# qq456cvb/VoteNet

Measured on AMD Instinct MI355X. Metric: SUN RGB-D 20k-pt scenes/sec (fwd+bwd), higher is better.
Workload: dtype f32

## Files before the change

### __graft_entry__.py

```python
import os
import sys

ROOT = os.path.dirname(os.path.abspath(__file__))
if ROOT not in sys.path:
    sys.path.insert(0, ROOT)


def build():
    import votenet_amd
    path = votenet_amd.build()
    from votenet_amd import _lib
    _lib.lib()
    _lib.monitors_lib()
    _lib.guard_lib()
    _lib.features_lib()
    _lib.detect_lib()
    _lib.boxpts_lib()
    _lib.aabb_lib()
    from oracle import oracle as O
    O.build()
    O.lib()
    print("built", path)


def smoke():
    import numpy as np
    import torch
    from oracle import oracle as O
    from votenet_amd import tf_grouping, tf_interpolate, tf_sampling
    assert torch.cuda.is_available(), "smoke() needs a GPU"
    dev = torch.device("cuda:0")
    xyz = np.random.default_rng(0).random((2, 2048, 3), dtype=np.float32)
    x = torch.from_numpy(xyz).to(dev)
    fidx = tf_sampling.farthest_point_sample(512, x)
    assert (fidx.cpu().numpy() == O.farthest_point_sample(512, xyz)).all(), "FPS indices differ from the oracle"
    new_xyz = tf_sampling.gather_point(x, fidx)
    idx, cnt = tf_grouping.query_ball_point(0.2, 32, x, new_xyz)
    oi, oc = O.query_ball_point(0.2, 32, xyz, new_xyz.cpu().numpy())
    assert (idx.cpu().numpy() == oi).all() and (cnt.cpu().numpy() == oc).all(), "ball query differs from the oracle"
    g = tf_grouping.group_point(x, idx)
    assert (g.cpu().numpy() == O.group_point(xyz, oi)).all(), "group_point differs from the oracle"
    dist, nn = tf_interpolate.three_nn(x, new_xyz)
    od, on = O.three_nn(xyz, new_xyz.cpu().numpy())
    assert (nn.cpu().numpy() == on).all() and (dist.cpu().numpy() == od).all(), "three_nn differs from the oracle"
    from votenet_amd import mlp
    rng = np.random.default_rng(1)
    w0 = (rng.normal(size=(6, 64)) * 0.5).astype(np.float32)
    w1 = (rng.normal(size=(64, 64)) * 0.2).astype(np.float32)
    ones, zeros = np.ones(64, np.float32), np.zeros(64, np.float32)
    a = O.group_concat(xyz, new_xyz.cpu().numpy(), xyz, oi).reshape(-1, 6)
    for w in (w0, w1):
        zz = O.linear(a, w, zeros)
        mean, var = O.bn_stats(zz)
        a = O.bn_relu(zz, mean, var, ones, zeros)
    exp = O.max_over_k(a, 32)
    T = lambda v: torch.from_numpy(v).to(dev)
    rows = 2 * 512 * 32
    z, st = mlp.linear_gather(x, new_xyz, x, idx, T(w0), T(zeros))
    sc, sh, _, _ = mlp.bn_finalize(rows, st, T(ones), T(zeros))
    z, st = mlp.linear_dense(z, T(w1), T(zeros), sc, sh, True)
    sc, sh, _, _ = mlp.bn_finalize(rows, st, T(ones), T(zeros))
    got, _ = mlp.bn_relu_max(z, 32, sc, sh, True)
    err = float(np.abs(got.cpu().numpy() - exp).max() / max(1.0, np.abs(exp).max()))
    assert err < 1e-5, "grouped MLP differs from the oracle: %g" % err
    z0, st0 = mlp.linear_gather(x, new_xyz, x, idx, T(w0), T(zeros))
    sc0, sh0, _, _ = mlp.bn_finalize(rows, st0, T(ones), T(zeros))
    w1d = T(w1)
    img = mlp.SplitImages([w1d])
    img.refresh()
    z3, st3 = mlp.linear_dense(z0, w1d, T(zeros), sc0, sh0, True)
    img.close()
# ... 37 lines not shown
```

### votenet_amd/_lib.py

```python
import ctypes
import os
import re
import subprocess

import torch

_HERE = os.path.dirname(os.path.abspath(__file__))
_LIB_PATH = os.path.join(_HERE, "lib", "libvotenet_hip.so")
_MON_PATH = os.path.join(_HERE, "lib", "libvotenet_monitors.so")
_GUARD_PATH = os.path.join(_HERE, "lib", "libvotenet_guard.so")
_FEAT_PATH = os.path.join(_HERE, "lib", "libvotenet_features.so")
_lib = None
_mon = None
_guard = None
_feat = None
_DETECT_PATH = os.path.join(_HERE, "lib", "libvotenet_detect.so")
_detect = None
_BOXPTS_PATH = os.path.join(_HERE, "lib", "libvotenet_boxpts.so")
_boxpts = None
_AABB_PATH = os.path.join(_HERE, "lib", "libvotenet_aabb.so")
_aabb = None


class VotenetError(RuntimeError):
    """A HIP runtime / launch / workspace error reported by libvotenet_hip.so."""


class InvalidArgumentError(ValueError):
    """Mirror of tf.errors.InvalidArgumentError raised by the reference's OP_REQUIRES checks."""


def lib_path():
    return _LIB_PATH


def build(force=False):
    if force:
        import glob
        mon = os.path.join(os.path.dirname(_LIB_PATH), os.path.basename(_MON_PATH))
        guard = os.path.join(os.path.dirname(_LIB_PATH), os.path.basename(_GUARD_PATH))
        feat = os.path.join(os.path.dirname(_LIB_PATH), os.path.basename(_FEAT_PATH))
        detect = os.path.join(os.path.dirname(_LIB_PATH), os.path.basename(_DETECT_PATH))
        boxpts = os.path.join(os.path.dirname(_LIB_PATH), os.path.basename(_BOXPTS_PATH))
        aabb = os.path.join(os.path.dirname(_LIB_PATH), os.path.basename(_AABB_PATH))
        for f in [_LIB_PATH, mon, guard, feat, detect, boxpts, aabb] + [o for d in ("obj", os.path.join("monitors", "obj"), os.path.join("guard", "obj"), os.path.join("features", "obj"),
                                                                               os.path.join("detect", "obj"), os.path.join("boxpts", "obj"), os.path.join("aabb", "obj"))
                                            for o in glob.glob(os.path.join(_HERE, "csrc", d, "*.o"))]:
            if os.path.exists(f):
                os.remove(f)
    out = subprocess.run(["bash", os.path.join(_HERE, "csrc", "build.sh")], capture_output=True, text=True)
    if out.returncode != 0:
        raise VotenetError("libvotenet_hip.so build failed:\n" + out.stdout + out.stderr)
    return _LIB_PATH


_SCALARS = {"int": ctypes.c_int, "long": ctypes.c_long, "float": ctypes.c_float, "double": ctypes.c_double, "unsigned": ctypes.c_uint,
            "unsigned long long": ctypes.c_ulonglong, "size_t": ctypes.c_size_t}
_POINTEES = set(_SCALARS) | {"void", "char", "unsigned char", "unsigned short", "long long"}


def _declarator(text, where):
    words = text.replace("*", " * ").split()
    if not words or not words[-1].isidentifier():
        raise ValueError("%s: cannot read the declaration '%s'" % (where, " ".join(text.split())))
    return " ".join(w for w in words[:-1] if w != "const" and w != "*"), words.count("*"), words[-1]


def _ctype(base, stars, structs, where, ret=False):
    if stars == 0 and base in _SCALARS:
        return _SCALARS[base]
    if stars == 0 and ret and base == "void":
        return None
    if stars == 1 and base in structs:
        return ctypes.POINTER(structs[base])
    if stars == 1 and ret and base == "char":
        return ctypes.c_char_p
    if stars == 1 and base in _POINTEES:
        return ctypes.c_void_p
    raise ValueError("%s: no ctypes type for the C type '%s'" % (where, base + " *" * stars))


def parse_header(text, structs):
    text = re.sub(r"/\*.*?\*/|//[^\n]*", " ", text, flags=re.S)
    text = re.sub(r"#ifdef __cplusplus.*?#endif", "", text, flags=re.S)
    text = re.sub(r"^[ \t]*#.*$", "", text, flags=re.M)

    def struct(m):
        name, fields = m.group(2), []
        for line in filter(str.strip, m.group(1).split(";")):
            decls = [_declarator(d, name) for d in line.split(",")]
            fields += [(n, _ctype(decls[0][0], stars, structs, name + "." + n)) for _, stars, n in decls]
        structs[name] = type("".join(w.capitalize() for w in name.split("_")[1:]), (ctypes.Structure,),
                             {"_fields_": fields, "__doc__": "struct %s of the C ABI." % name})
        return ""
    text = re.sub(r"typedef\s+struct\s+\w+\s*\{(.*?)\}\s*(\w+)\s*;", struct, text, flags=re.S)
    funcs = {}
    for stmt in text.split(";"):
        if not stmt.strip():
            continue
# ... 102 lines not shown
            fn.restype, fn.argtypes = restype, argtypes
        _feat = F
    return _feat


def detect_lib():
    global _detect
    if _detect is None:
        if not os.path.exists(_DETECT_PATH):
            raise VotenetError("libvotenet_detect.so not found at %s -- run `python -c 'import __graft_entry__ as g; g.build()'` "
                               "(there is no CPU fallback)" % _DETECT_PATH)
        with open(os.path.join(_HERE, os.pardir, "include", "votenet_detections.h")) as f:
            protos = parse_header(f.read(), {})
        D = ctypes.CDLL(_DETECT_PATH)
        for name, (restype, argtypes) in protos.items():
            fn = getattr(D, name)
            fn.restype, fn.argtypes = restype, argtypes
        _detect = D
    return _detect


def boxpts_lib():
    global _boxpts
    if _boxpts is None:
        if not os.path.exists(_BOXPTS_PATH):
            raise VotenetError("libvotenet_boxpts.so not found at %s -- run `python -c 'import __graft_entry__ as g; g.build()'` "
                               "(there is no CPU fallback)" % _BOXPTS_PATH)
        with open(os.path.join(_HERE, os.pardir, "include", "votenet_box_points.h")) as f:
            protos = parse_header(f.read(), {})
        B = ctypes.CDLL(_BOXPTS_PATH)
        for name, (restype, argtypes) in protos.items():
            fn = getattr(B, name)
            fn.restype, fn.argtypes = restype, argtypes
        _boxpts = B
    return _boxpts


def aabb_lib():
    global _aabb
    if _aabb is None:
        if not os.path.exists(_AABB_PATH):
            raise VotenetError("libvotenet_aabb.so not found at %s -- run `python -c 'import __graft_entry__ as g; g.build()'` "
                               "(there is no CPU fallback)" % _AABB_PATH)
        with open(os.path.join(_HERE, os.pardir, "include", "votenet_aabb_nms.h")) as f:
            protos = parse_header(f.read(), {})
        A = ctypes.CDLL(_AABB_PATH)
        for name, (restype, argtypes) in protos.items():
            fn = getattr(A, name)
            fn.restype, fn.argtypes = restype, argtypes
        _aabb = A
    return _aabb


def check_aabb(rc):
    if rc == 0:
        return
    msg = aabb_lib().votenet_aabb_last_error().decode()
    if rc == 1:
        raise InvalidArgumentError(msg)
    raise VotenetError("libvotenet_aabb error %d: %s" % (rc, msg))


def check_boxpts(rc):
    if rc == 0:
        return
    msg = boxpts_lib().votenet_box_points_last_error().decode()
    if rc == 1:
        raise InvalidArgumentError(msg)
    raise VotenetError("libvotenet_boxpts error %d: %s" % (rc, msg))


def check_detect(rc):
    if rc == 0:
        return
    msg = detect_lib().votenet_detections_last_error().decode()
    if rc == 1:
        raise InvalidArgumentError(msg)
    raise VotenetError("libvotenet_detect error %d: %s" % (rc, msg))


def check_features(rc):
    if rc == 0:
        return
    msg = features_lib().votenet_point_features_last_error().decode()
    if rc == 1:
        raise InvalidArgumentError(msg)
    raise VotenetError("libvotenet_features error %d: %s" % (rc, msg))


def check_guard(rc):
    if rc == 0:
        return
    msg = guard_lib().votenet_step_guard_last_error().decode()
    if rc == 1:
        raise InvalidArgumentError(msg)
    raise VotenetError("libvotenet_guard error %d: %s" % (rc, msg))


def check_monitors(rc):
    if rc == 0:
        return
    msg = monitors_lib().votenet_monitors_last_error().decode()
    if rc == 1:
        raise InvalidArgumentError(msg)
    raise VotenetError("libvotenet_monitors error %d: %s" % (rc, msg))

# ... 67 lines not shown
```

### votenet_amd/csrc/grouping.hip

```cpp
#include "common.h"
#include <cmath>

namespace votenet {


template <int NW, int G = 8>
__global__ __launch_bounds__(NW * 64) void ball_query_kernel(int n, int m, float thr, int nsample,
                                                              const float *__restrict__ xyz1,
                                                              const float *__restrict__ xyz2, int *__restrict__ idx,
                                                              int *__restrict__ pts_cnt)
{
    constexpr int WPQ = NW * G;
    constexpr int CHUNK = WPQ * 32;
    constexpr int QPW = 64 / NW;
    constexpr int LPQ = WPQ / 64 > 0 ? WPQ / 64 : 1;
    __shared__ unsigned masks[64][WPQ + 1];

    const int scene = blockIdx.y;
    const float *__restrict__ cand = xyz1 + (size_t)scene * n * 3;
    const float *__restrict__ qry = xyz2 + (size_t)scene * m * 3;
    int *__restrict__ oidx = idx + (size_t)scene * m * nsample;
    int *__restrict__ ocnt = pts_cnt + (size_t)scene * m;

    const int lane = lane_id();
    const int w = wave_id_uniform();
    const int q0 = blockIdx.x * 64;
    const int q = q0 + lane;
    const bool qvalid = q < m;
    const int qq = qvalid ? q : (m - 1);
    const float qx = qry[(size_t)qq * 3 + 0], qy = qry[(size_t)qq * 3 + 1], qz = qry[(size_t)qq * 3 + 2];

    int cnt[QPW];
    int first[QPW];
#pragma unroll
    for (int i = 0; i < QPW; i++) {
        cnt[i] = 0;
        first[i] = 0;
    }

    for (int base = 0; base < n; base += CHUNK) {
#pragma unroll 1
        for (int g = 0; g < G; g++) {
            const int wbase = __builtin_amdgcn_readfirstlane(base + (w * G + g) * 32);
            unsigned mask = 0;
            if (wbase < n) {
                const int valid = (n - wbase) < 32 ? (n - wbase) : 32;
                if (valid == 32) {
#pragma unroll
                    for (int t = 0; t < 32; t++) {
                        const float cx = cand[(size_t)(wbase + t) * 3 + 0];
                        const float cy = cand[(size_t)(wbase + t) * 3 + 1];
                        const float cz = cand[(size_t)(wbase + t) * 3 + 2];
                        const float dx = qx - cx, dy = qy - cy, dz = qz - cz;
// ... 59 lines not shown
            if (cnt[i] < nsample && q0 + ql < m) wave_full = false;
        }
        if (__syncthreads_and(wave_full ? 1 : 0)) break;
    }
#pragma unroll
    for (int i = 0; i < QPW; i++) {
        const int ql = w * QPW + i;
        if (q0 + ql < m) {
            const int c = cnt[i] < nsample ? cnt[i] : nsample;
            int *__restrict__ row = oidx + (size_t)(q0 + ql) * nsample;
            for (int l = c + lane; l < nsample; l += 64) row[l] = first[i];
            if (lane == 0) ocnt[q0 + ql] = c;
        }
    }
}

__global__ void group_point_vec4_kernel(long rows, int n, int c4, long rows_per_scene, const float4 *__restrict__ points,
                                        const int *__restrict__ idx, float4 *__restrict__ out)
{
    const long total = rows * c4;
    for (long e = (long)blockIdx.x * blockDim.x + threadIdx.x; e < total; e += (long)gridDim.x * blockDim.x) {
        const long row = e / c4;
        const int v = (int)(e - row * c4);
        const long s = row / rows_per_scene;
        const int ii = idx[row];
        out[e] = points[((size_t)s * n + ii) * c4 + v];
    }
}

__global__ void group_point_kernel(long rows, int n, int c, long rows_per_scene, const float *__restrict__ points,
                                   const int *__restrict__ idx, float *__restrict__ out)
{
    const long total = rows * c;
    for (long e = (long)blockIdx.x * blockDim.x + threadIdx.x; e < total; e += (long)gridDim.x * blockDim.x) {
        const long row = e / c;
        const int l = (int)(e - row * c);
        const long s = row / rows_per_scene;
        const int ii = idx[row];
        out[e] = points[((size_t)s * n + ii) * c + l];
    }
}

__global__ void group_point_grad_kernel(long rows, int n, int c, long rows_per_scene, const float *__restrict__ grad_out,
                                        const int *__restrict__ idx, float *__restrict__ grad_points)
{
    const long total = rows * c;
    for (long e = (long)blockIdx.x * blockDim.x + threadIdx.x; e < total; e += (long)gridDim.x * blockDim.x) {
        const long row = e / c;
        const int l = (int)(e - row * c);
        const long s = row / rows_per_scene;
        const int ii = idx[row];
        unsafeAtomicAdd(&grad_points[((size_t)s * n + ii) * c + l], grad_out[e]);
    }
}

float ball_threshold(float r)
{
    float t = r * r;
    while (t > 0.0f && sqrtf(t) >= r) t = nextafterf(t, 0.0f);
    while (sqrtf(t) < r) t = nextafterf(t, INFINITY);
    return t;
}

static inline int grid_for(long total, int block)
{
    long g = (total + block - 1) / block;
    if (g > 256 * 16) g = 256 * 16;
    if (g < 1) g = 1;
    return (int)g;
}

}

using namespace votenet;

extern "C" float votenet_ball_threshold(float radius) { return ball_threshold(radius); }

static int g_bq_small = 0;
extern "C" void votenet_debug_ball_query_small(int form) { VN_DEBUG_GATE(); g_bq_small = form; }

extern "C" int votenet_query_ball_point(int b, int n, int m, float radius, int nsample, const float *xyz1,
                                        const float *xyz2, int *idx, int *pts_cnt, void *stream)
{
    VN_REQUIRE(radius > 0, "QueryBallPoint expects positive radius");
    VN_REQUIRE(nsample > 0, "QueryBallPoint expects positive nsample");
    VN_REQUIRE(b >= 0 && n > 0, "QueryBallPoint expects (batch_size, ndataset, 3) xyz1 shape.");
    VN_REQUIRE(m >= 0, "QueryBallPoint expects (batch_size, npoint, 3) xyz2 shape.");
    if (b == 0 || m == 0) return VOTENET_OK;
    VN_REQUIRE(xyz1 && xyz2 && idx && pts_cnt, "QueryBallPoint: null buffer");
    const float thr = (radius <= 1e-20f) ? -1.0f : ball_threshold(radius);
    hipStream_t st = as_stream(stream);
    dim3 grid((m + 63) / 64, b);
    if (n > 2048 || g_bq_small == 16)
        hipLaunchKernelGGL((ball_query_kernel<16>), grid, dim3(1024), 0, st, n, m, thr, nsample, xyz1, xyz2, idx, pts_cnt);
    else if (g_bq_small == 4)
        hipLaunchKernelGGL((ball_query_kernel<4>), grid, dim3(256), 0, st, n, m, thr, nsample, xyz1, xyz2, idx, pts_cnt);
    else if (n > 1024)
        hipLaunchKernelGGL((ball_query_kernel<16, 4>), grid, dim3(1024), 0, st, n, m, thr, nsample, xyz1, xyz2, idx, pts_cnt);
    else if (n > 512)
        hipLaunchKernelGGL((ball_query_kernel<16, 2>), grid, dim3(1024), 0, st, n, m, thr, nsample, xyz1, xyz2, idx, pts_cnt);
    else
        hipLaunchKernelGGL((ball_query_kernel<16, 1>), grid, dim3(1024), 0, st, n, m, thr, nsample, xyz1, xyz2, idx, pts_cnt);
    return check_launch("query_ball_point");
}

namespace votenet {
constexpr int BQI_CH = 6;
constexpr int BQI_U = 6;
template <int WAVES>
__global__ __launch_bounds__(WAVES * 64) void ball_query_indexed_kernel(int n, int m, float thr, int nsample,
                                                                        const float *__restrict__ xyz2, const int *__restrict__ perm,
                                                                        const float *__restrict__ bbox,
                                                                        const float4 *__restrict__ sorted, int *__restrict__ idx,
                                                                        int *__restrict__ pts_cnt)
// ... 173 lines not shown
```

### votenet_amd/mlp.py

```python
import ctypes

import torch

from . import _lib as L

PROFILE_EVENTS = None
PROFILE_SHAPES = None


class _Timed:
    def __init__(self, kind, flops, shape=None, limit=None):
        self.kind, self.flops, self.shape = kind, flops, shape
        if limit is not None and getattr(limit, "nh_limit", None) is not None:
            self.flops = (flops, limit.nh_dev, BALL_PIECES * limit.G)

    def __enter__(self):
        if PROFILE_EVENTS is not None:
            self.e0, self.e1 = torch.cuda.Event(enable_timing=True), torch.cuda.Event(enable_timing=True)
            self.e0.record()

    def __exit__(self, *a):
        if PROFILE_EVENTS is not None:
            self.e1.record()
            PROFILE_EVENTS.append((self.e0, self.e1, self.kind, self.flops) if PROFILE_SHAPES is None else (self.e0, self.e1, self.kind, self.flops, self.shape))
# ... 520 lines not shown


def assemble_rows_half(xyz, new_xyz, idx, pts_cnt, half):
    b, m, k = idx.shape
    n = xyz.shape[1]
    if k != 64:
        raise L.InvalidArgumentError("assemble_rows_half expects nsample == 64")
    geo = torch.empty((b * m * 64, 4), dtype=torch.float32, device=xyz.device)
    npts = b * n
    nz = npts * 4 + 16 + (npts + 1) // 2
    if half.nh_limit is not None and _StatsArena.active and _StatsArena.whole_step:
        zero = _zeros_i64((nz,), xyz.device)
    else:
        zero = torch.zeros(nz, dtype=torch.int64, device=xyz.device)
    cntv = zero[:npts * 4].view(npts, 4)
    mom = zero[npts * 4:npts * 4 + 9].view(torch.float64)
    work = zero[npts * 4 + 16:].view(torch.int32)[:npts]
    with L.device_guard(xyz.device):
        L.check(L.lib().votenet_assemble_rows_half(b, n, m, L.ptr(half.nh_dev), L.ptr(xyz), L.ptr(new_xyz), L.ptr(idx), L.ptr(pts_cnt),
                                                   L.ptr(half._hc), L.ptr(geo), L.ptr(cntv), L.ptr(mom), L.ptr(work), L.stream_ptr()))
    half._geo, half._work = geo, work
    return geo, cntv, mom


def narrow_rows_half(xyz, new_xyz, feat, idx, pts_cnt, half):
    b, m, k = idx.shape
    n = xyz.shape[1]
    c = feat.shape[2] if feat is not None else 0
    if k != 64:
        raise L.InvalidArgumentError("narrow_rows_half expects nsample == 64")
    u8 = torch.empty((b * m * 64, 8), dtype=torch.float32, device=xyz.device)
    mom = torch.zeros(72, dtype=torch.float64, device=xyz.device)
    with L.device_guard(xyz.device):
        L.check(L.lib().votenet_narrow_rows_half(b, n, m, c, L.ptr(half.nh_dev), L.ptr(xyz), L.ptr(new_xyz), L.ptr(feat), L.ptr(idx),
                                                 L.ptr(pts_cnt), L.ptr(half._hc), L.ptr(u8), L.ptr(mom), L.stream_ptr()))
    half._u8 = u8
    return u8, mom


def half_sort_rows(half, npts):
    dev = half._geo.device
    work, half._work = getattr(half, "_work", None), None
    counted = work is not None
    if not counted:
        work = torch.empty(npts, dtype=torch.int32, device=dev)
    order = torch.empty(half.G * 64, dtype=torch.int32, device=dev)
    with L.device_guard(dev):
        L.check(L.lib().votenet_half_sort_rows(npts, half.G, L.ptr(half.nh_dev), L.ptr(half._geo), L.ptr(work), 1 if counted else 0, L.ptr(order),
                                               L.stream_ptr()))
    half._order = order
    if half.nh is not None:
        half.order = order[:half.nh * PIECE]
    return order


def group_linear_backward_half(half, b, n, P, wx, da, coef, relu, dw_xyz):
    cout = P.shape[1]
    if getattr(half, "order", None) is None:
        half_sort_rows(half, b * n)
    S = _zeros_f32((b, n, cout), P.device)
    with L.device_guard(P.device):
        L.check(L.lib().votenet_group_linear_backward_sorted(half.nh, cout, L.ptr(half.order), L.ptr(half.geo), L.ptr(half.wh), L.ptr(P),
                                                             L.ptr(wx), L.ptr(da), L.ptr(coef), 1 if relu else 0, L.ptr(S), L.ptr(dw_xyz),
                                                             L.ptr(half.nh_limit), L.stream_ptr()))
    return S


_masked_slots = None


def dgrad_bn_half(z, coef, relu, wT, da, half):
    rows, c = z.shape
    cout = wT.shape[1]
    out = torch.empty((rows, cout), dtype=torch.float32, device=z.device)
    with L.device_guard(z.device), _Timed("linear_dense", 2.0 * rows * c * cout, (rows, c, cout, "dgrad_bn half"), limit=half):
        L.check(L.lib().votenet_mlp_dgrad_bn_half(rows, c, cout, L.ptr(da), L.ptr(z), L.ptr(coef), 1 if relu else 0, L.ptr(wT), L.ptr(out),
                                                  L.ptr(half.wh), L.ptr(half.nh_limit), L.stream_ptr()))
    return out


def group_linear_backward_decomposed(half, b, n, P, wx, da, bn, relu, tail, cntv, mom, dw_xyz, eps=BN_EPS, defer=None):
    cout = P.shape[1]
    dev = P.device
    if getattr(half, "order", None) is None:
        half_sort_rows(half, b * n)
    sc, sh, me, va = bn
    global _masked_slots, COEF_TAIL
    if _masked_slots is None:
        _masked_slots = int(L.lib().votenet_group_linear_backward_masked_slots())
    nparts = _masked_slots
    S = _zeros_f32((b, n, cout), dev)
    small = _zeros_f32((3 + 3 * nparts, cout), dev)
    ug, vp = small[:3], small[3:]
    zeros = _zeros_f64(2 * cout + _masked_slots * 5 * cout, dev)
    sums, part = zeros[:2 * cout], zeros[2 * cout:]
    prev_ct, COEF_TAIL = COEF_TAIL, True
    try:
        t, coef = _coef_tail(tail, cout, dev)
    finally:
        COEF_TAIL = prev_ct
    with L.device_guard(dev):
        L.check(L.lib().votenet_group_linear_backward_masked(half.nh, cout, L.ptr(half.order), L.ptr(half.geo), L.ptr(P), L.ptr(wx), L.ptr(da),
                                                             L.ptr(sc), L.ptr(sh), L.ptr(me), L.ptr(va), eps, 1 if relu else 0, L.ptr(S),
                                                             L.ptr(ug), L.ptr(sums), L.ptr(part), ctypes.byref(t), L.ptr(half.nh_limit),
                                                             L.stream_ptr()))
        L.check(L.lib().votenet_assembled_point_grad(b * n, cout, L.ptr(P), L.ptr(cntv), L.ptr(wx), L.ptr(coef), L.ptr(S), L.ptr(vp),
# ... 767 lines not shown
```

### votenet_amd/model.py

```python

import math

import torch

from . import checkpoint
from . import dp
from . import mlp as M
from . import pointnet2 as P

NH, NS, NC = 12, 10, 10
PREFETCH_AFTER = 2
SIDE_PRIORITY = 0
WGRAD_PRIORITY = 0
PROPOSAL_NUM = 256
PROPOSAL_OUT = 5 + 2 * NH + 4 * NS + NC
LEARNING_RATE = 1e-3


GEOMETRY_GRAPHS = True
GEOMETRY_MAX_EVICTIONS = 8
GEOMETRY_RING = 3


class GeometryGraph:
# ... 659 lines not shown

    def _stretch_eligible(self, x, cot, gt):
        return bool(STRETCH_GRAPH and gt is not None and cot is None and x.is_cuda and not M.DETERMINISTIC and PREFETCH_AFTER < 5
                    and M.PROFILE_EVENTS is None and P._FROZEN.table is None and not getattr(self, "_stretch_off", False)
                    and not torch.cuda.is_current_stream_capturing())

    @staticmethod
    def _stretch_inputs(lv, g):
        ins = dict(lv)
        for name in ("fp1", "fp2"):
            idx, w = g[name]
            ins[name + "_idx"], ins[name + "_w"] = idx, w
            inv = getattr(idx, "_inv", None)
            if inv is not None:
                ins[name + "_inv0"], ins[name + "_inv1"] = inv
        ins["prop_fps"] = g["prop_fps"]
        return ins

    def _stretch_body(self, I, tape_levels, wgrad_stream, gt=None, cut=None, loss_hook=None, copy_seeds=False):
        from . import loss as VL

        def geom(name):
            idx = I[name + "_idx"]
            if name + "_inv0" in I:
                idx._inv = (I[name + "_inv0"], I[name + "_inv1"])
            return idx, I[name + "_w"]
        tail = []
        lv = {k: I[k] for k in ("l2_xyz", "l2_p", "l3_xyz", "l3_p", "l4_xyz", "l4_p")}
        out = self._head_forward(lv, geom("fp1"), geom("fp2"), I["prop_fps"], tail, copy_seeds=copy_seeds)
        self.update_moving_averages(list(tape_levels) + tail)
        losses, cot = loss_hook(out) if loss_hook is not None else VL.votenet_loss(out, gt)
        if loss_hook is None and self.monitors is not None:
            self.last_accuracies = self.monitors.after_loss(out, gt, losses)
        with P.WGRAD.on(wgrad_stream):
            grads = self._head_backward(tail, cot, cut=cut)
            if cut is None:
                P.wgrad_join()
        self._stretch_tail = tail
        return out, losses, grads

    def _train_step_stretch(self, x, gt, tape, next_x, feats=None, next_feats=None):
        self.store.refresh_split()
        lv, g = self.backbone_levels(x, tape, next_x=next_x, feats=feats, next_feats=next_feats)
        self._stamp_tape(tape)
        self._grams_ahead(tape)
        if not all(k in g for k in ("fp1", "fp2", "prop_fps")):
            g = dict(g)
            g.setdefault("fp1", P.FPModule.geometry(lv["l3_xyz"], lv["l4_xyz"]))
            g.setdefault("fp2", P.FPModule.geometry(lv["l2_xyz"], lv["l3_xyz"]))
            g.setdefault("prop_fps", P.tf_sampling.farthest_point_sample(self.proposal.npoint, lv["l2_xyz"]))
        ins = self._stretch_inputs(lv, g)
        key = tuple((k, tuple(v.shape), v.dtype) for k, v in ins.items()) + (P.HALF_GROUPS, P.ASSEMBLE_FIRST, P.ASSEMBLE_INLINE, P.POOL_GRAM_BACKWARD, P.ASSEMBLED_DECOMPOSED,
                                                                             self.overlap_wgrad, STRETCH_SEGMENTS, M.SPLIT_K, M.COEF_TAIL, P.WGRAD_BATCH, P.POOL_IN_EPILOGUE,
                                                                             self.store.split, bool(getattr(self, "inline_wgrad_tail", INLINE_WGRAD_TAIL)), M.FORWARD_H2, M.ADHOC_H2, M.CONFIG_EPOCH)
        graphs = self.__dict__.setdefault("_stretch_graphs", {})
        sg = graphs.get(key)
        self._gsync.begin()
        if sg is None:
            dkey = key[:-1]
            demand = self.__dict__.setdefault("_stretch_demand", {}).get(dkey)
            geometry_events = P.tf_sampling.PROFILE_EVENTS is not None or P.tf_grouping.PROFILE_EVENTS is not None
            if demand is None or geometry_events:
                a = M._StatsArena
                off0, want0 = a.off, a.want32
                self.check_tape(tape)
                out, self.last_losses, grads = self._stretch_body(ins, tape, self._wgrad_side(), gt=gt,
                                                                  copy_seeds=getattr(self, "_geometry_current", None) is not None)
                self._stretch_demand[dkey] = (a.off - off0, a.want32 - want0)
                self._backward_levels_pass(tape, grads)
                return out
            while len(graphs) >= STRETCH_MAX_GRAPHS:
                graphs.pop(min(graphs, key=lambda k: graphs[k].last_used))
            sg = graphs[key] = StretchGraph(self, ins, tape, demand)
        self._stretch_clock = getattr(self, "_stretch_clock", 0) + 1
        sg.last_used = self._stretch_clock
        self.store._fresh_wait()
        mon = self.monitors
        out, self.last_losses, grads = sg.replay(ins, gt, self._wgrad_side(),
                                                 after_loss=mon.after_loss if mon is not None else None)
        if mon is not None:
            self.last_accuracies = mon.accuracies
        self._ema_version += 1
        self._backward_levels_pass(tape, grads)
        return out

    def _grams_early(self, levels):
        if not GRAM_EARLY or M.DETERMINISTIC or P.WGRAD.stream is None:
            return
        todo = [levels[n]["recs"][-1] for n in GRAM_EARLY if n in levels]
        todo = [r for r in todo if r.get("gram_form") and r.get("in_affine") is not None and "gram_ahead" not in r]
        if not todo:
            return

        def run():
            for r in todo:
                r["gram_ahead"] = M.gram(r["x"], r["in_affine"][:2], r["in_relu"], half=r.get("half"))
        P.on_wgrad_stream(run, *[r["x"] for r in todo])
        P.wgrad_flush()

    def _grams_ahead(self, tape):
        if not GRAMS_AHEAD or M.DETERMINISTIC or not self.overlap_wgrad or not torch.cuda.is_available():
            return
        todo = [t["recs"][-1] for t in tape[:4] if t.get("op") == "sa" and t["recs"][-1].get("gram_form") and t["recs"][-1].get("in_affine") is not None]
        if not todo:
            return

        def run():
# ... 120 lines not shown
```

### votenet_amd/pointnet2.py

```python
import math
import threading

import torch

from . import mlp as M
from . import tf_grouping, tf_interpolate, tf_sampling


PAD_RAGGED = True
NARROW_FIRST = True
PAD_RAGGED_IN = True
ASSEMBLE_FIRST = True
ASSEMBLE_INLINE = True
HALF_GROUPS = True
FUSE_BN_REDUCE = True


class ParamStore:

    def __init__(self, device):
        self.device = device
        self._specs = []
        self.flat = None
        self.grad = None
# ... 641 lines not shown
    return M.attach_inverse(idx, xyz.shape[1]), cnt


def sample_and_group(npoint, radius, nsample, xyz, sample_xyz=None, knn=False):
    fps_idx = tf_sampling.farthest_point_sample(npoint, sample_xyz if sample_xyz is not None else xyz)
    new_xyz = tf_sampling.gather_point(xyz, fps_idx)
    idx, pts_cnt = _group_indices(radius, nsample, xyz, new_xyz, knn)
    return fps_idx, new_xyz, idx, pts_cnt


POOLINGS = ("max", "avg", "weighted_avg", "max_and_avg")


class SAModule:

    def __init__(self, store, scope, npoint, radius, nsample, cin, mlp, mlp2=None, knn=False, prefix="conv", leaf=False, pooling="max",
                 group_all=False):
        if pooling not in POOLINGS:
            raise ValueError("SAModule: pooling must be one of %s, got %r" % (", ".join(POOLINGS), pooling))
        self.pooling, self.group_all = pooling, bool(group_all)
        self.plain_pool = self.group_all or pooling != "max"
        if self.group_all:
            npoint, radius, nsample, knn = 1, None, None, False
        self.npoint, self.radius, self.nsample, self.knn = npoint, radius, nsample, knn
        self.leaf, self.cin = leaf, cin
        self.mlp = make_mlp(store, scope, 3 + cin, mlp, prefix)
        store.want_transpose(self.mlp[0].name + "/W", 3, None)
        store._split_rows.append((self.mlp[0].name + "/W", 3, None))
        store.want_transpose(self.mlp[0].name + "/W", 0, 3)
        pooled = 2 * mlp[-1] if pooling == "max_and_avg" else mlp[-1]
        self.mlp2 = make_mlp(store, scope, pooled, mlp2, "conv_post_", last_plain=True) if mlp2 else None

    def narrow(self, rows):
        m = self.mlp
        return bool(NARROW_FIRST and not self.plain_pool and self.leaf and len(m) >= 3 and m[0].bn and m[1].bn and m[0].relu and
                    M.narrow_supported(rows, 3 + self.cin, m[0].cout, m[1].cout))

    def assembled(self, b, n):
        m = self.mlp
        if self.plain_pool:
            return False
        rows = b * self.npoint * self.nsample
        return bool(ASSEMBLE_FIRST and PRE_LINEAR and not M.DETERMINISTIC and self.cin > 0 and not self.narrow(rows) and len(m) >= 3
                    and m[0].bn and m[1].bn and m[0].relu and M.assembled_supported(rows, m[0].cout, m[1].cout)
                    and M.group_linear_backward_supported(m[0].cout, self.nsample) and b * n * m[0].cout * 4 < 2 ** 32)

    def half_groups(self, b, n):
        m = self.mlp
        if not (HALF_GROUPS and not self.plain_pool and not M.DETERMINISTIC and not self.knn and self.nsample == 64 and len(m) == 3 and m[2].bn and POOL_IN_EPILOGUE
                and POOL_GRAM_BACKWARD and (b * self.npoint) % 8 == 0 and M.pool_backward_supported(m[1].cout, m[2].cout, 64)):
            return False
        return bool(self.narrow(b * self.npoint * 64) or (m[1].cout == 128 and self.assembled(b, n)))

    def geometry(self, xyz, sample_xyz=None, fps_idx=None, points=None, ahead=True):
        if fps_idx is None:
            geom = sample_and_group(self.npoint, self.radius, self.nsample, xyz, sample_xyz, self.knn)
        else:
            new_xyz = tf_sampling.gather_point(xyz, fps_idx)
            idx, pts_cnt = _group_indices(self.radius, self.nsample, xyz, new_xyz, self.knn)
            geom = (fps_idx, new_xyz, idx, pts_cnt)
        if (points is not None or self.cin == 0) and self.narrow(xyz.shape[0] * self.npoint * self.nsample):
            if ahead and self.half_groups(xyz.shape[0], xyz.shape[1]):
                half = M.half_groups(geom[3])
                geom = tuple(geom) + M.narrow_rows_half(xyz, geom[1], points, geom[2], geom[3], half) + (half,)
            else:
                geom = tuple(geom) + M.narrow_rows(xyz, geom[1], points, geom[2])
        elif (ahead or ASSEMBLE_INLINE) and self.half_groups(xyz.shape[0], xyz.shape[1]):
            half = M.half_groups(geom[3], device_count=not ahead)
            geom = tuple(geom) + M.assemble_rows_half(xyz, geom[1], geom[2], geom[3], half) + (half,)
            M.half_sort_rows(half, xyz.shape[0] * xyz.shape[1])
        elif self.assembled(xyz.shape[0], xyz.shape[1]) and (ahead or ASSEMBLE_INLINE):
            geom = tuple(geom) + M.assemble_rows(xyz, geom[1], geom[2], pts_cnt=geom[3], in_pass=not ahead)
        return geom

    def forward(self, xyz, points, sample_xyz=None, tape=None, geom=None):
        if self.plain_pool:
            return self._forward_plain_pool(xyz, points, sample_xyz, tape, geom)
        b = xyz.shape[0]
        geom = geom if geom is not None else self.geometry(xyz, sample_xyz, points=points)
        fps_idx, new_xyz, idx, pts_cnt = geom[:4]
        recs = []
        rows = b * self.npoint * self.nsample
        first = ("gather", xyz, new_xyz, points, idx)
        if self.narrow(rows):
            u8, mom = geom[4:6] if len(geom) >= 6 else M.narrow_rows(xyz, new_xyz, points, idx)
            first = ("narrow", u8, mom)
            if len(geom) >= 7:
                half = geom[6].resolve()
                first = ("narrow", half.u8, mom, half)
        elif points is not None and self.assembled(b, xyz.shape[1]) and (len(geom) >= 7 or ASSEMBLE_INLINE):
            geo, cntv, mom = geom[4:7] if len(geom) >= 7 else M.assemble_rows(xyz, new_xyz, idx, pts_cnt=pts_cnt, in_pass=True)
            first = ("assembled", xyz, new_xyz, points, idx, geo, cntv, mom)
            if len(geom) >= 8:
                half = geom[7].resolve()
                first = ("assembled", xyz, new_xyz, points, idx, half.geo, cntv, mom, half)
        z, pend = mlp_chain_forward(self.mlp, rows, first, recs, pool_k=self.nsample, keep_z=tape is not None)
        if recs[-1]["pool"] is not None:
            res = M.bn_pool_finalize(recs[-1]["pool"], None, None, True, want_argmax=tape is not None, bn=pend,
                                     want_zsel=tape is not None and bool(recs[-1].get("gram_form")), half=recs[-1].get("half"))
            pooled, argmax, zsel = res if len(res) == 3 else (res[0], res[1], None)
        else:
            zsel = None
            sc, sh = pend.finalize()
            pooled, argmax = M.bn_relu_max(z, self.nsample, sc, sh, True, want_argmax=tape is not None)
        recs2 = []
        out = pooled
        if self.mlp2:
# ... 220 lines not shown
```

Measured before the change: 2345.

## Fuse vote grouping: gather, ball query and half-layout assembly in two kernels

Adds a dedicated library that runs the proposal-module vote grouping (gather of sampled centres, ball query with 64 samples, and the half-group row layout with geometry, counts, moments and scatter order) in two kernels instead of the existing chain of separate ops. The ball query uses per-wave bitmasks in shared memory and stops early once every query is full. The layout kernel builds one scene per block in shared memory. It targets launch count and intermediate traffic for small vote sets (n,m <=1024), at the cost of a large new code path with tight shared-memory limits.

```diff
diff --git a/__graft_entry__.py b/__graft_entry__.py
--- a/__graft_entry__.py
+++ b/__graft_entry__.py
@@ -17,6 +17,7 @@
     _lib.detect_lib()
     _lib.boxpts_lib()
     _lib.aabb_lib()
+    _lib.groupvotes_lib()
     from oracle import oracle as O
     O.build()
     O.lib()
diff --git a/include/votenet_group_votes.h b/include/votenet_group_votes.h
--- /dev/null
+++ b/include/votenet_group_votes.h
@@ -0,0 +1,20 @@
+#ifndef VOTENET_GROUP_VOTES_H
+#define VOTENET_GROUP_VOTES_H
+
+#ifdef __cplusplus
+extern "C" {
+#endif
+
+const char *votenet_group_votes_last_error(void);
+
+int votenet_group_votes_supported(int b, int n, int m, int nsample);
+
+int votenet_group_votes(int b, int n, int m, float radius, int nsample, const float *xyz, const int *inds, float *new_xyz, int *idx,
+                        int *pts_cnt, int *pos, int *hc, float *wh, int *nh_dev, float *geo, long long *cntv, double *mom, int *count,
+                        int *order, void *stream);
+
+#ifdef __cplusplus
+}
+#endif
+
+#endif
diff --git a/votenet_amd/_lib.py b/votenet_amd/_lib.py
--- a/votenet_amd/_lib.py
+++ b/votenet_amd/_lib.py
@@ -20,6 +20,8 @@
 _boxpts = None
 _AABB_PATH = os.path.join(_HERE, "lib", "libvotenet_aabb.so")
 _aabb = None
+_GROUPVOTES_PATH = os.path.join(_HERE, "lib", "libvotenet_groupvotes.so")
+_groupvotes = None
 
 
 class VotenetError(RuntimeError):
@@ -43,8 +45,10 @@
         detect = os.path.join(os.path.dirname(_LIB_PATH), os.path.basename(_DETECT_PATH))
         boxpts = os.path.join(os.path.dirname(_LIB_PATH), os.path.basename(_BOXPTS_PATH))
         aabb = os.path.join(os.path.dirname(_LIB_PATH), os.path.basename(_AABB_PATH))
-        for f in [_LIB_PATH, mon, guard, feat, detect, boxpts, aabb] + [o for d in ("obj", os.path.join("monitors", "obj"), os.path.join("guard", "obj"), os.path.join("features", "obj"),
-                                                                               os.path.join("detect", "obj"), os.path.join("boxpts", "obj"), os.path.join("aabb", "obj"))
+        groupvotes = os.path.join(os.path.dirname(_LIB_PATH), os.path.basename(_GROUPVOTES_PATH))
+        for f in [_LIB_PATH, mon, guard, feat, detect, boxpts, aabb, groupvotes] + [o for d in ("obj", os.path.join("monitors", "obj"), os.path.join("guard", "obj"), os.path.join("features", "obj"),
+                                                                               os.path.join("detect", "obj"), os.path.join("boxpts", "obj"), os.path.join("aabb", "obj"),
+                                                                               os.path.join("groupvotes", "obj"))
                                             for o in glob.glob(os.path.join(_HERE, "csrc", d, "*.o"))]:
             if os.path.exists(f):
                 os.remove(f)
@@ -253,6 +257,31 @@
     return _aabb
 
 
+def groupvotes_lib():
+    global _groupvotes
+    if _groupvotes is None:
+        if not os.path.exists(_GROUPVOTES_PATH):
+            raise VotenetError("libvotenet_groupvotes.so not found at %s -- run `python -c 'import __graft_entry__ as g; g.build()'` "
+                               "(there is no CPU fallback)" % _GROUPVOTES_PATH)
+        with open(os.path.join(_HERE, os.pardir, "include", "votenet_group_votes.h")) as f:
+            protos = parse_header(f.read(), {})
+        V = ctypes.CDLL(_GROUPVOTES_PATH)
+        for name, (restype, argtypes) in protos.items():
+            fn = getattr(V, name)
+            fn.restype, fn.argtypes = restype, argtypes
+        _groupvotes = V
+    return _groupvotes
+
+
+def check_groupvotes(rc):
+    if rc == 0:
+        return
+    msg = groupvotes_lib().votenet_group_votes_last_error().decode()
+    if rc == 1:
+        raise InvalidArgumentError(msg)
+    raise VotenetError("libvotenet_groupvotes error %d: %s" % (rc, msg))
+
+
 def check_aabb(rc):
     if rc == 0:
         return
diff --git a/votenet_amd/csrc/ball_threshold.h b/votenet_amd/csrc/ball_threshold.h
--- /dev/null
+++ b/votenet_amd/csrc/ball_threshold.h
@@ -0,0 +1,14 @@
+#pragma once
+#include <cmath>
+
+namespace votenet {
+
+inline float ball_threshold(float r)
+{
+    float t = r * r;
+    while (t > 0.0f && sqrtf(t) >= r) t = nextafterf(t, 0.0f);
+    while (sqrtf(t) < r) t = nextafterf(t, INFINITY);
+    return t;
+}
+
+}
diff --git a/votenet_amd/csrc/grouping.hip b/votenet_amd/csrc/grouping.hip
--- a/votenet_amd/csrc/grouping.hip
+++ b/votenet_amd/csrc/grouping.hip
@@ -1,4 +1,5 @@
 #include "common.h"
+#include "ball_threshold.h"
 #include <cmath>
 
 namespace votenet {
@@ -164,14 +165,6 @@
         const int ii = idx[row];
         unsafeAtomicAdd(&grad_points[((size_t)s * n + ii) * c + l], grad_out[e]);
     }
-}
-
-float ball_threshold(float r)
-{
-    float t = r * r;
-    while (t > 0.0f && sqrtf(t) >= r) t = nextafterf(t, 0.0f);
-    while (sqrtf(t) < r) t = nextafterf(t, INFINITY);
-    return t;
 }
 
 static inline int grid_for(long total, int block)
diff --git a/votenet_amd/csrc/groupvotes/group_votes.hip b/votenet_amd/csrc/groupvotes/group_votes.hip
--- /dev/null
+++ b/votenet_amd/csrc/groupvotes/group_votes.hip
@@ -0,0 +1,403 @@
+#include "../mlp_types.h"
+#include "../ball_threshold.h"
+
+#include <cstdint>
+#pragma GCC visibility push(default)
+#include "../../../include/votenet_group_votes.h"
+#pragma GCC visibility pop
+
+namespace votenet {
+
+static thread_local char g_gv_err[512] = "";
+static int gv_set_error(int code, const char *fmt, ...)
+{
+    va_list ap;
+    va_start(ap, fmt);
+    vsnprintf(g_gv_err, sizeof(g_gv_err), fmt, ap);
+    va_end(ap);
+    return code;
+}
+#define GV_REQUIRE(cond, ...)                                                              \
+    do {                                                                                   \
+        if (!(cond)) return ::votenet::gv_set_error(VOTENET_E_INVALID_ARGUMENT, __VA_ARGS__); \
+    } while (0)
+
+constexpr int PS = kPiece, NP = kBallPieces, TP = kTilePieces;
+constexpr int GV_K = 64;
+constexpr int GV_MAX_B = 65535;
+constexpr int GV_MAX_N = 1024;
+constexpr int GV_MAX_M = 1024;
+static_assert(PS * NP == GV_K, "a ball is NP pieces of PS rows");
+
+__device__ __forceinline__ int gv_kept_pieces(int cnt)
+{
+    const int c = cnt < 1 ? 1 : cnt;
+    const int k = (c + PS - 1) / PS;
+    return k > NP ? NP : k;
+}
+__device__ __forceinline__ double gv_shfl_xor_f64(double v, int m)
+{
+    int lo = __double2loint(v), hi = __double2hiint(v);
+    lo = __shfl_xor(lo, m);
+    hi = __shfl_xor(hi, m);
+    return __hiloint2double(hi, lo);
+}
+__device__ __forceinline__ long long gv_fixed(float v) { return (long long)((double)v * 4294967296.0); }
+
+template <int G>
+__global__ __launch_bounds__(1024) void gv_ball_query_kernel(int n, int m, float thr, const float *__restrict__ xyz,
+                                                             const int *__restrict__ inds, float *__restrict__ new_xyz,
+                                                             int *__restrict__ idx, int *__restrict__ pts_cnt)
+{
+    constexpr int NW = 16;
+    constexpr int WPQ = NW * G;
+    constexpr int CHUNK = WPQ * 32;
+    constexpr int QPW = 64 / NW;
+    constexpr int nsample = GV_K;
+    static_assert(WPQ <= 64, "the pop phase reads one mask word per lane");
+    __shared__ unsigned masks[64][WPQ + 1];
+
+    const int scene = blockIdx.y;
+    const float *__restrict__ cand = xyz + (size_t)scene * n * 3;
+    int *__restrict__ oidx = idx + (size_t)scene * m * nsample;
+    int *__restrict__ ocnt = pts_cnt + (size_t)scene * m;
+
+    const int lane = lane_id();
+    const int w = wave_id_uniform();
+    const int q0 = blockIdx.x * 64;
+    const int q = q0 + lane;
+    const bool qvalid = q < m;
+    const int qq = qvalid ? q : (m - 1);
+    int a = inds[(size_t)scene * m + qq];
+    a = a < 0 ? 0 : (a >= n ? n - 1 : a);
+    const float qx = cand[(size_t)a * 3 + 0], qy = cand[(size_t)a * 3 + 1], qz = cand[(size_t)a * 3 + 2];
+    if (w == 0 && qvalid) {
+        float *__restrict__ o = new_xyz + ((size_t)scene * m + q) * 3;
+        o[0] = qx;
+        o[1] = qy;
+        o[2] = qz;
+    }
+
+    int cnt[QPW];
+    int first[QPW];
+#pragma unroll
+    for (int i = 0; i < QPW; i++) {
+        cnt[i] = 0;
+        first[i] = 0;
+    }
+
+    for (int base = 0; base < n; base += CHUNK) {
+#pragma unroll 1
+        for (int g = 0; g < G; g++) {
+            const int wbase = __builtin_amdgcn_readfirstlane(base + (w * G + g) * 32);
+            unsigned mask = 0;
+            if (wbase < n) {
+                const int valid = (n - wbase) < 32 ? (n - wbase) : 32;
+                if (valid == 32) {
+#pragma unroll
+                    for (int t = 0; t < 32; t++) {
+                        const float cx = cand[(size_t)(wbase + t) * 3 + 0];
+                        const float cy = cand[(size_t)(wbase + t) * 3 + 1];
+                        const float cz = cand[(size_t)(wbase + t) * 3 + 2];
+                        const float dx = qx - cx, dy = qy - cy, dz = qz - cz;
+                        const float s = dx * dx + dy * dy + dz * dz;
+                        mask |= (s < thr ? 1u : 0u) << t;
+                    }
+                } else {
+                    for (int t = 0; t < valid; t++) {
+                        const float cx = cand[(size_t)(wbase + t) * 3 + 0];
+                        const float cy = cand[(size_t)(wbase + t) * 3 + 1];
+                        const float cz = cand[(size_t)(wbase + t) * 3 + 2];
+                        const float dx = qx - cx, dy = qy - cy, dz = qz - cz;
+                        const float s = dx * dx + dy * dy + dz * dz;
+                        mask |= (s < thr ? 1u : 0u) << t;
+                    }
+                }
+            }
+            masks[lane][w * G + g] = mask;
+        }
+        __syncthreads();
+        bool wave_full = true;
+#pragma unroll
+        for (int i = 0; i < QPW; i++) {
+            const int ql = w * QPW + i;
+            if (cnt[i] < nsample && q0 + ql < m) {
+                unsigned long long bits = lane < WPQ ? (unsigned long long)masks[ql][lane] : 0ull;
+                const int cbase = base + lane * 32;
+                const int pc = __popcll(bits);
+                int incl = pc;
+#pragma unroll
+                for (int d = 1; d < 64; d <<= 1) {
+                    const int t = __shfl_up(incl, d);
+                    if (lane >= d) incl += t;
+                }
+                const int total = __builtin_amdgcn_readlane(incl, 63);
+                if (total > 0) {
+                    if (cnt[i] == 0) {
+                        const unsigned long long have = __ballot(pc > 0);
+                        const int fl = __ffsll((long long)have) - 1;
+                        const int mine = cbase + (bits ? __ffsll((long long)bits) - 1 : 0);
+                        first[i] = __builtin_amdgcn_readlane(mine, fl);
+                    }
+                    int pos = cnt[i] + incl - pc;
+                    int *__restrict__ row = oidx + (size_t)(q0 + ql) * nsample;
+                    while (bits && pos < nsample) {
+                        const int t = __ffsll((long long)bits) - 1;
+                        row[pos] = cbase + t;
+                        pos++;
+                        bits &= bits - 1;
+                    }
+                    cnt[i] += total;
+                }
+            }
+            if (cnt[i] < nsample && q0 + ql < m) wave_full = false;
+        }
+        if (__syncthreads_and(wave_full ? 1 : 0)) break;
+    }
+#pragma unroll
+    for (int i = 0; i < QPW; i++) {
+        const int ql = w * QPW + i;
+        if (q0 + ql < m) {
+            const int c = cnt[i] < nsample ? cnt[i] : nsample;
+            int *__restrict__ row = oidx + (size_t)(q0 + ql) * nsample;
+            for (int l = c + lane; l < nsample; l += 64) row[l] = first[i];
+            if (lane == 0) ocnt[q0 + ql] = c;
+        }
+    }
+}
+
+__global__ __launch_bounds__(1024) void gv_layout_kernel(int n, int m, int G, const float *__restrict__ xyz,
+                                                         const float *__restrict__ new_xyz, const int *__restrict__ idx,
+                                                         const int *__restrict__ pts_cnt, int *__restrict__ pos, int *__restrict__ hc,
+                                                         float *__restrict__ wh, int *__restrict__ nh_out, float4 *__restrict__ geo,
+                                                         long long *__restrict__ cntv, double *__restrict__ mom, int *__restrict__ count,
+                                                         int *__restrict__ order)
+{
+    __shared__ unsigned long long s_cntv[GV_MAX_N * 4];
+    __shared__ float s_xyz[GV_MAX_N * 3];
+    __shared__ int s_count[GV_MAX_N];
+    __shared__ int s_pos[GV_MAX_M * (NP - 1)];
+    __shared__ int s_wave[16], s_before[16], s_total[16];
+    __shared__ double s_mom[16][9];
+    const int scene = blockIdx.x, tid = threadIdx.x, lane = tid & 63;
+    const int wv = wave_id_uniform();
+    const int c_lo = scene * m;
+
+    for (int e = tid; e < n * 4; e += 1024) s_cntv[e] = 0ull;
+    for (int e = tid; e < n; e += 1024) s_count[e] = 0;
+    for (int e = tid; e < n * 3; e += 1024) s_xyz[e] = xyz[(size_t)scene * n * 3 + e];
+
+    int before = 0, total = 0;
+    for (int c = tid; c < G; c += 1024) {
+        const int e = gv_kept_pieces(pts_cnt[c]) - 1;
+        total += e;
+        before += c < c_lo ? e : 0;
+    }
+#pragma unroll
+    for (int off = 32; off >= 1; off >>= 1) {
+        before += __shfl_xor(before, off);
+        total += __shfl_xor(total, off);
+    }
+    if (lane == 0) {
+        s_before[wv] = before;
+        s_total[wv] = total;
+    }
+    __syncthreads();
+    before = total = 0;
+#pragma unroll
+    for (int w = 0; w < 16; w++) {
+        before += s_before[w];
+        total += s_total[w];
+    }
+    const int E = total;
+    const int P = (TP - (G + E) % TP) % TP;
+    const int nh = G + E + P;
+    if (scene == 0 && tid == 0) nh_out[0] = nh;
+
+    int carry = before;
+    for (int l0 = 0; l0 < m; l0 += 1024) {
+        const int cl = l0 + tid;
+        const bool own = cl < m;
+        const int c = c_lo + (own ? cl : 0);
+        const int kc = own ? gv_kept_pieces(pts_cnt[c]) : 1;
+        const int mine = kc - 1;
+        int x = mine;
+#pragma unroll
+        for (int off = 1; off < 64; off <<= 1) {
+            const int t = __shfl_up(x, off);
+            if (lane >= off) x += t;
+        }
+        __syncthreads();
+        if (lane == 63) s_wave[wv] = x;
+        __syncthreads();
+        int base = carry;
+        for (int w = 0; w < wv; w++) base += s_wave[w];
+        for (int w = 0; w < 16; w++) carry += s_wave[w];
+        if (own) {
+            const int p = base + x - mine;
+            const int f = 3 * c - p;
+            int npad = P - f;
+            npad = npad < 0 ? 0 : (npad > NP - kc ? NP - kc : npad);
+            hc[c] = c * NP;
+            wh[c] = 1.0f + (float)(PS * (NP - (kc + npad)));
+#pragma unroll
+            for (int j = 1; j < NP; j++) {
+                int pj = -1;
+                if (j < kc) pj = p + (j - 1);
+                else if (j - kc < npad) pj = E + f + (j - kc);
+                if (pj >= 0) {
+                    hc[G + pj] = c * NP + j;
+                    wh[G + pj] = 1.0f;
+                }
+                pos[(size_t)c * (NP - 1) + j - 1] = pj;
+                s_pos[cl * (NP - 1) + j - 1] = pj;
+            }
+        }
+    }
+    __syncthreads();
+
+    int fb = 3 * c_lo - before;
+    fb = fb < P ? fb : P;
+    const int rows_before = PS * (c_lo + before + fb);
+
+    const int k = lane, j = k / PS, s = k % PS;
+    const int nit = (m + 15) / 16;
+    double acc[9];
+#pragma unroll
+    for (int i = 0; i < 9; i++) acc[i] = 0.0;
+    for (int it0 = 0; it0 < nit; it0 += 4) {
+        int id4[4], cnt4[4], q4[4];
+        float cx[4], cy[4], cz[4];
+#pragma unroll
+        for (int u = 0; u < 4; u++) {
+            const int cl = (it0 + u) * 16 + wv;
+            const bool own = cl < m;
+            const int cc = own ? cl : 0;
+            const int c = c_lo + cc;
+            const int pj = j == 0 ? 0 : s_pos[cc * (NP - 1) + (j == 0 ? 0 : j - 1)];
+            q4[u] = !own ? -1 : (j == 0 ? c : (pj >= 0 ? G + pj : -1));
+            id4[u] = idx[(size_t)c * GV_K + k];
+            cnt4[u] = pts_cnt[c];
+            cx[u] = new_xyz[(size_t)c * 3 + 0];
+            cy[u] = new_xyz[(size_t)c * 3 + 1];
+            cz[u] = new_xyz[(size_t)c * 3 + 2];
+        }
+#pragma unroll
+        for (int u = 0; u < 4; u++) {
+            if (q4[u] < 0) continue;
+            int id = id4[u];
+            id = id < 0 ? 0 : (id >= n ? n - 1 : id);
+            const unsigned prow = (unsigned)scene * (unsigned)n + (unsigned)id;
+            const float dx = s_xyz[id * 3 + 0] - cx[u];
+            const float dy = s_xyz[id * 3 + 1] - cy[u];
+            const float dz = s_xyz[id * 3 + 2] - cz[u];
+            geo[(size_t)q4[u] * PS + s] = make_float4(dx, dy, dz, __uint_as_float(prow));
+            atomicAdd(&s_count[id], 1);
+            const int cnt = cnt4[u] < 1 ? 1 : cnt4[u];
+            if (k < cnt) {
+                const long long mult = (k == 0) ? (long long)(GV_K - cnt + 1) : 1LL;
+                atomicAdd(&s_cntv[id * 4 + 0], (unsigned long long)mult);
+                atomicAdd(&s_cntv[id * 4 + 1], (unsigned long long)(mult * gv_fixed(dx)));
+                atomicAdd(&s_cntv[id * 4 + 2], (unsigned long long)(mult * gv_fixed(dy)));
+                atomicAdd(&s_cntv[id * 4 + 3], (unsigned long long)(mult * gv_fixed(dz)));
+                const double mu = (double)mult, x = dx, y = dy, z = dz;
+                acc[0] += mu * x; acc[1] += mu * y; acc[2] += mu * z;
+                acc[3] += mu * x * x; acc[4] += mu * x * y; acc[5] += mu * x * z; acc[6] += mu * y * y; acc[7] += mu * y * z; acc[8] += mu * z * z;
+            }
+        }
+    }
+#pragma unroll
+    for (int i = 0; i < 9; i++) {
+        double v = acc[i];
+#pragma unroll
+        for (int mk = 32; mk >= 1; mk >>= 1) v += gv_shfl_xor_f64(v, mk);
+        if (lane == 0) s_mom[wv][i] = v;
+    }
+    __syncthreads();
+    if (tid < 9) {
+        double v = 0.0;
+        for (int w = 0; w < 16; w++) v += s_mom[w][tid];
+        unsafeAtomicAdd(&mom[tid], v);
+    }
+
+    {
+        const int v = tid < n ? s_count[tid] : 0;
+        int x = v;
+#pragma unroll
+        for (int off = 1; off < 64; off <<= 1) {
+            const int t = __shfl_up(x, off);
+            if (lane >= off) x += t;
+        }
+        if (lane == 63) s_wave[wv] = x;
+        __syncthreads();
+        int start = rows_before + x - v;
+        for (int w = 0; w < wv; w++) start += s_wave[w];
+        if (tid < n) {
+            s_count[tid] = start;
+            count[(size_t)scene * n + tid] = start + v;
+        }
+        unsigned long long *__restrict__ cv = reinterpret_cast<unsigned long long *>(cntv) + (size_t)scene * n * 4;
+        for (int e = tid; e < n * 4; e += 1024) cv[e] = s_cntv[e];
+    }
+    __syncthreads();
+
+    for (int it0 = 0; it0 < nit; it0 += 4) {
+        int id4[4], q4[4];
+#pragma unroll
+        for (int u = 0; u < 4; u++) {
+            const int cl = (it0 + u) * 16 + wv;
+            const bool own = cl < m;
+            const int cc = own ? cl : 0;
+            const int c = c_lo + cc;
+            const int pj = j == 0 ? 0 : s_pos[cc * (NP - 1) + (j == 0 ? 0 : j - 1)];
+            q4[u] = !own ? -1 : (j == 0 ? c : (pj >= 0 ? G + pj : -1));
+            id4[u] = idx[(size_t)c * GV_K + k];
+        }
+#pragma unroll
+        for (int u = 0; u < 4; u++) {
+            if (q4[u] < 0) continue;
+            int id = id4[u];
+            id = id < 0 ? 0 : (id >= n ? n - 1 : id);
+            const int slot = atomicAdd(&s_count[id], 1);
+            order[slot] = q4[u] * PS + s;
+        }
+    }
+
+    const long max_rows = (long)GV_K * G;
+    for (long r = (long)nh * PS + (long)blockIdx.x * 1024 + tid; r < max_rows; r += (long)gridDim.x * 1024)
+        geo[r] = make_float4(0.f, 0.f, 0.f, __uint_as_float(0u));
+}
+
+}
+
+using namespace votenet;
+
+extern "C" const char *votenet_group_votes_last_error(void) { return g_gv_err; }
+
+extern "C" int votenet_group_votes_supported(int b, int n, int m, int nsample)
+{
+    return (b >= 1 && b <= GV_MAX_B && n >= 1 && n <= GV_MAX_N && m >= 1 && m <= GV_MAX_M && nsample == GV_K && ((long)b * m) % TP == 0) ? 1 : 0;
+}
+
+extern "C" int votenet_group_votes(int b, int n, int m, float radius, int nsample, const float *xyz, const int *inds, float *new_xyz,
+                                   int *idx, int *pts_cnt, int *pos, int *hc, float *wh, int *nh_dev, float *geo, long long *cntv,
+                                   double *mom, int *count, int *order, void *stream)
+{
+    GV_REQUIRE(votenet_group_votes_supported(b, n, m, nsample),
+               "group_votes serves 1 <= b <= %d scenes, 1 <= n <= %d candidates, 1 <= m <= %d centres, nsample == %d, (b m) %% %d == 0; got b = %d, "
+               "n = %d, m = %d, nsample = %d", GV_MAX_B, GV_MAX_N, GV_MAX_M, GV_K, TP, b, n, m, nsample);
+    GV_REQUIRE(radius > 0, "group_votes expects a positive radius");
+    GV_REQUIRE(xyz && inds && new_xyz && idx && pts_cnt && pos && hc && wh && nh_dev && geo && cntv && mom && count && order,
+               "group_votes: null buffer");
+    GV_REQUIRE((uintptr_t)geo % 16 == 0 && (uintptr_t)cntv % 16 == 0, "group_votes: geo / cntv must be 16-byte aligned");
+    const float thr = (radius <= 1e-20f) ? -1.0f : ball_threshold(radius);
+    hipStream_t st = as_stream(stream);
+    const dim3 grid((m + 63) / 64, b);
+    if (n > 512) hipLaunchKernelGGL((gv_ball_query_kernel<2>), grid, dim3(1024), 0, st, n, m, thr, xyz, inds, new_xyz, idx, pts_cnt);
+    else hipLaunchKernelGGL((gv_ball_query_kernel<1>), grid, dim3(1024), 0, st, n, m, thr, xyz, inds, new_xyz, idx, pts_cnt);
+    hipLaunchKernelGGL(gv_layout_kernel, dim3(b), dim3(1024), 0, st, n, m, b * m, xyz, new_xyz, idx, pts_cnt, pos, hc, wh, nh_dev,
+                       reinterpret_cast<float4 *>(geo), cntv, mom, count, order);
+    const hipError_t e = hipGetLastError();
+    if (e != hipSuccess) return gv_set_error(VOTENET_E_HIP, "group_votes: %s", hipGetErrorString(e));
+    return VOTENET_OK;
+}
diff --git a/votenet_amd/mlp.py b/votenet_amd/mlp.py
--- a/votenet_amd/mlp.py
+++ b/votenet_amd/mlp.py
@@ -596,6 +596,40 @@
     if half.nh is not None:
         half.order = order[:half.nh * PIECE]
     return order
+
+
+GROUP_VOTES = True
+
+
+def group_votes_supported(b, n, m, nsample):
+    return bool(GROUP_VOTES and L.groupvotes_lib().votenet_group_votes_supported(int(b), int(n), int(m), int(nsample)))
+
+
+def group_votes(xyz, inds, radius, nsample=64):
+    b, n = xyz.shape[:2]
+    m = inds.shape[1]
+    G, npts, dev = b * m, b * n, xyz.device
+    new_xyz = torch.empty((b, m, 3), dtype=torch.float32, device=dev)
+    idx = torch.empty((b, m, 64), dtype=torch.int32, device=dev)
+    ints = torch.empty(G + (BALL_PIECES - 1) * G + BALL_PIECES * G + 1 + npts + 64 * G, dtype=torch.int32, device=dev)
+    o = 0
+    pts_cnt, o = ints[o:o + G].view(b, m), o + G
+    pos, o = ints[o:o + (BALL_PIECES - 1) * G], o + (BALL_PIECES - 1) * G
+    hc, o = ints[o:o + BALL_PIECES * G], o + BALL_PIECES * G
+    nh, o = ints[o:o + 1], o + 1
+    count, o = ints[o:o + npts], o + npts
+    order = ints[o:]
+    wh = torch.empty(BALL_PIECES * G, dtype=torch.float32, device=dev)
+    geo = torch.empty((G * 64, 4), dtype=torch.float32, device=dev)
+    cntv = torch.empty((npts, 4), dtype=torch.int64, device=dev)
+    mom = (_zeros_f64(16, dev) if _StatsArena.active and _StatsArena.whole_step else torch.zeros(16, dtype=torch.float64, device=dev))[:9]
+    with L.device_guard(dev):
+        L.check_groupvotes(L.groupvotes_lib().votenet_group_votes(b, n, m, float(radius), int(nsample), L.ptr(xyz), L.ptr(inds), L.ptr(new_xyz),
+                                                                  L.ptr(idx), L.ptr(pts_cnt), L.ptr(pos), L.ptr(hc), L.ptr(wh), L.ptr(nh),
+                                                                  L.ptr(geo), L.ptr(cntv), L.ptr(mom), L.ptr(count), L.ptr(order), L.stream_ptr()))
+        half = HalfLayout(G, pos, hc, wh, nh, device_count=True)
+    half._geo, half._order, half._work, half._ends = geo, order, None, count
+    return new_xyz, idx, pts_cnt, geo, cntv, mom, half
 
 
 def group_linear_backward_half(half, b, n, P, wx, da, coef, relu, dw_xyz):
diff --git a/votenet_amd/model.py b/votenet_amd/model.py
--- a/votenet_amd/model.py
+++ b/votenet_amd/model.py
@@ -735,7 +735,7 @@
         ins = self._stretch_inputs(lv, g)
         key = tuple((k, tuple(v.shape), v.dtype) for k, v in ins.items()) + (P.HALF_GROUPS, P.ASSEMBLE_FIRST, P.ASSEMBLE_INLINE, P.POOL_GRAM_BACKWARD, P.ASSEMBLED_DECOMPOSED,
                                                                              self.overlap_wgrad, STRETCH_SEGMENTS, M.SPLIT_K, M.COEF_TAIL, P.WGRAD_BATCH, P.POOL_IN_EPILOGUE,
-                                                                             self.store.split, bool(getattr(self, "inline_wgrad_tail", INLINE_WGRAD_TAIL)), M.FORWARD_H2, M.ADHOC_H2, M.CONFIG_EPOCH)
+                                                                             self.store.split, bool(getattr(self, "inline_wgrad_tail", INLINE_WGRAD_TAIL)), M.FORWARD_H2, M.ADHOC_H2, M.GROUP_VOTES, M.CONFIG_EPOCH)
         graphs = self.__dict__.setdefault("_stretch_graphs", {})
         sg = graphs.get(key)
         self._gsync.begin()
diff --git a/votenet_amd/pointnet2.py b/votenet_amd/pointnet2.py
--- a/votenet_amd/pointnet2.py
+++ b/votenet_amd/pointnet2.py
@@ -717,7 +717,21 @@
             return False
         return bool(self.narrow(b * self.npoint * 64) or (m[1].cout == 128 and self.assembled(b, n)))
 
+    def _group_votes(self, xyz, fps_idx, points):
+        if not (M.GROUP_VOTES and ASSEMBLE_INLINE and tf_sampling.PROFILE_EVENTS is None and tf_grouping.PROFILE_EVENTS is None):
+            return False
+        b, n = xyz.shape[:2]
+        if (points is not None or self.cin == 0) and self.narrow(b * self.npoint * self.nsample):
+            return False
+        if not (xyz.is_cuda and xyz.dtype == torch.float32 and xyz.is_contiguous() and fps_idx.dtype == torch.int32 and fps_idx.is_contiguous()
+                and tuple(fps_idx.shape) == (b, self.npoint) and self.radius is not None and float(self.radius) > 0):
+            return False
+        return bool(self.half_groups(b, n) and M.group_votes_supported(b, n, self.npoint, self.nsample))
+
     def geometry(self, xyz, sample_xyz=None, fps_idx=None, points=None, ahead=True):
+        if fps_idx is not None and not ahead and self._group_votes(xyz, fps_idx, points):
+            new_xyz, idx, pts_cnt, geo, cntv, mom, half = M.group_votes(xyz, fps_idx, self.radius, self.nsample)
+            return (fps_idx, new_xyz, idx, pts_cnt, geo, cntv, mom, half)
         if fps_idx is None:
             geom = sample_and_group(self.npoint, self.radius, self.nsample, xyz, sample_xyz, self.knn)
         else:
```

New measurement: 2362, median of 5. Within noise of the previous version (+0.7%).
